# wangtong627/COR

Hardware: AMD Instinct MI355X
Metric: query triplets/sec (forward + similarity + top-k) (higher is better)
Workload: dtype bf16

## Files before the change

### cor_amd/csrc/flash_attn.hip

```cpp
#include <cstdlib>
#include <type_traits>

#include "common.h"

typedef short s16x4 __attribute__((ext_vector_type(4)));

namespace {

struct FlashArgs {
  const bf16_t* q; const bf16_t* k; const bf16_t* v; void* o;
  long q_sb, q_st, k_sb, k_st, v_sb, v_st, o_sb, o_st;
  int H, Tq, Tk;
  float scale_log2;
  float tbl_scale;
  const bf16_t* pad_row; const float* rel_h; const float* rel_w;
  int grid, S, nW, d3;
  int nqt;
  int rev;
};

constexpr int KT = 64;
constexpr int TILE_B = KT * 128;
constexpr int KV_BYTES = 4 * TILE_B;
constexpr int AUX_PER_WAVE = 8192;
// ... 717 lines not shown
  const int wi_ = a.rev ? (int)gridDim.x - 1 - wi0_ : wi0_;
  const int qt_ = wi_ % a.nqt, hb_ = wi_ / a.nqt;
  const int head = hb_ % a.H, b = hb_ / a.H;
  constexpr int S = 64;
  const int g2 = S * S;
  const bf16_t* kvbase = a.q + (long)b * g2 * a.d3 + head * 64;
  const int qh = qt_ * NW + wave;

  u32x4 qf[2][4];
#pragma unroll
  for (int qb = 0; qb < 2; ++qb) {
    const bf16_t* qp = a.q + ((long)b * g2 + qh * S + qb * 32 + r) * a.d3 + head * 64;
#pragma unroll
    for (int c = 0; c < 4; ++c) qf[qb][c] = *(const u32x4*)(qp + 16 * c + 8 * h);
  }

  float* aux = (float*)(smem + K_BYTES + V_BYTES + wave * AUXW);
  f32x16 wreg[2][2];
  {
    float* scr = (float*)(smem + wave * (3 * 4096));
    uint4 fh[2][4], fw[4][4];
#pragma unroll
    for (int kb = 0; kb < 2; ++kb)
#pragma unroll
      for (int c = 0; c < 4; ++c) fh[kb][c] = table_frag(a.rel_h, qh + (S - 1) - (kb * 32 + r), c, h);
#pragma unroll
    for (int jb = 0; jb < 4; ++jb)
#pragma unroll
      for (int c = 0; c < 4; ++c) fw[jb][c] = table_frag(a.rel_w, min(jb * 32 + r, 2 * S - 2), c, h);
#pragma unroll
    for (int qb = 0; qb < 2; ++qb) {
#pragma unroll
      for (int kb = 0; kb < 2; ++kb) {
        f32x16 acc;
#pragma unroll
        for (int e = 0; e < 16; ++e) acc[e] = 0.f;
#pragma unroll
        for (int c = 0; c < 4; ++c)
          acc = __builtin_amdgcn_mfma_f32_32x32x16_bf16(__builtin_bit_cast(bf16x8, fh[kb][c]), __builtin_bit_cast(bf16x8, qf[qb][c]), acc, 0, 0, 0);
#pragma unroll
        for (int e = 0; e < 16; ++e) aux[(kb * 32 + acc_row(e, h)) * 64 + qb * 32 + r] = acc[e] * a.tbl_scale;
      }
#pragma unroll
      for (int jb = 0; jb < 3; ++jb) {
        f32x16 acc;
#pragma unroll
        for (int e = 0; e < 16; ++e) acc[e] = 0.f;
#pragma unroll
        for (int c = 0; c < 4; ++c)
          acc = __builtin_amdgcn_mfma_f32_32x32x16_bf16(__builtin_bit_cast(bf16x8, fw[qb + jb][c]), __builtin_bit_cast(bf16x8, qf[qb][c]), acc, 0, 0, 0);
#pragma unroll
        for (int e = 0; e < 16; ++e) scr[(jb * 32 + acc_row(e, h)) * 32 + r] = acc[e] * a.tbl_scale;
      }
      __builtin_amdgcn_fence(__ATOMIC_ACQ_REL, "wavefront");
#pragma unroll
      for (int kb = 0; kb < 2; ++kb)
#pragma unroll
        for (int e = 0; e < 16; ++e) wreg[qb][kb][e] = scr[(r + (S - 1) - (kb * 32 + acc_row(e, h))) * 32 + r];
      __builtin_amdgcn_fence(__ATOMIC_ACQ_REL, "wavefront");
    }
  }
  __syncthreads();

  char* Kring = smem; char* Vring = smem + K_BYTES;
  const unsigned lds0 = __builtin_amdgcn_readfirstlane((unsigned)(size_t)((__attribute__((address_space(3))) char*)smem));
  const unsigned wofs = __builtin_amdgcn_readfirstlane(wave) * 1024u;
  const int nt = a.Tk / KT;
  const int srow = tid >> 3, sch = tid & 7;
  const int kswz = (sch ^ ((srow >> 1) & 7)) * 8;
  const int vswz = (sch ^ (((srow >> 1) & 1) << 2)) * 8;
  const unsigned vk0 = (unsigned)((srow * a.d3 + a.H * 64 + kswz) * 2), vk1 = vk0 + (unsigned)(32 * a.d3 * 2);
  const unsigned vv0 = (unsigned)((srow * a.d3 + 2 * a.H * 64 + vswz) * 2), vv1 = vv0 + (unsigned)(32 * a.d3 * 2);
  const long tile_bytes = (long)KT * a.d3 * 2;
  auto issue_k = [&](int t, int slot) {
    const char* base = (const char*)kvbase + (long)t * tile_bytes;
    const unsigned d = lds0 + slot * TILE_B + wofs;
    glds16_so(base, vk0, d);
    glds16_so(base, vk1, d + 4096);
  };
  auto issue_v = [&](int t, int slot) {
    const char* base = (const char*)kvbase + (long)t * tile_bytes;
    const unsigned d = lds0 + K_BYTES + slot * TILE_B + wofs;
    glds16_so(base, vv0, d);
    glds16_so(base, vv1, d + 4096);
  };
  issue_k(0, 0); issue_k(1, 1); issue_k(2, 2); issue_v(0, 0); issue_v(1, 1);
  *(uint4*)(Vring + 3 * TILE_B + tid * 16) = make_uint4(0, 0, 0, 0);
  *(uint4*)(Vring + 3 * TILE_B + 4096 + tid * 16) = make_uint4(0, 0, 0, 0);
  asm volatile("s_waitcnt vmcnt(0)" ::: "memory");
  __syncthreads();

  const int sw = (lane >> 1) & 7;
  int kch[4];
#pragma unroll
  for (int c = 0; c < 4; ++c) kch[c] = r * 128 + (((2 * c + h) ^ sw) << 4);
  const int v_tr = (4 * h + ((lane & 15) >> 2)) * 128 + (16 * ((lane >> 4) & 1) + 4 * (lane & 3)) * 2;
  const int v_trd[2] = {v_tr + ((lane >> 3) & 1) * 64, v_tr + (1 - ((lane >> 3) & 1)) * 64};

  f32x16 o[2][2], s[2][2];
  float lsum[2][2] = {{0.f, 0.f}, {0.f, 0.f}};
  float m[2] = {-INFINITY, -INFINITY};
  u32x4 pf[2][2][2];
#pragma unroll
  for (int qb = 0; qb < 2; ++qb)
#pragma unroll
    for (int x = 0; x < 2; ++x) {
#pragma unroll
      for (int e = 0; e < 16; ++e) o[qb][x][e] = 0.f;
      pf[qb][x][0] = u32x4{0, 0, 0, 0}; pf[qb][x][1] = u32x4{0, 0, 0, 0};
    }

  {
    uint4 kf[8];
#pragma unroll
    for (int i = 0; i < 8; ++i) kf[i] = *(const uint4*)(Kring + (i >> 2) * 32 * 128 + kch[i & 3]);
#pragma unroll
    for (int qb = 0; qb < 2; ++qb)
#pragma unroll
      for (int kb = 0; kb < 2; ++kb) {
        s[qb][kb] = wreg[qb][kb];
#pragma unroll
        for (int c = 0; c < 4; ++c)
          s[qb][kb] = __builtin_amdgcn_mfma_f32_32x32x16_bf16(__builtin_bit_cast(bf16x8, kf[kb * 4 + c]), __builtin_bit_cast(bf16x8, qf[qb][c]), s[qb][kb], 0, 0, 0);
      }
  }
  __syncthreads();

#pragma unroll
  for (int qb = 0; qb < 2; ++qb) {
#pragma unroll
    for (int c = 0; c < 4; ++c) asm volatile("" : "+a"(qf[qb][c]));
#pragma unroll
    for (int x = 0; x < 2; ++x) { asm volatile("" : "+v"(s[qb][x])); asm volatile("" : "+v"(wreg[qb][x])); asm volatile("" : "+a"(o[qb][x])); }
  }
  const char* ksrc = (const char*)kvbase + 3 * tile_bytes;
  const char* vsrc = (const char*)kvbase + 2 * tile_bytes;
  const unsigned vk0p = vk0 + 2048u, vk1p = vk1 - 2048u, vv0p = vv0 + 2048u, vv1p = vv1 - 2048u;

#pragma unroll 1
  for (int t = 0; t < nt; ++t) {
    auto dma_tile = [&](const unsigned dst, const unsigned v0, const unsigned v1, const char* src) __attribute__((always_inline)) {
      unsigned keep;
      asm volatile("s_mov_b32 %0, m0\n\ts_mov_b32 m0, %1\n\ts_nop 0\n\t"
                   "global_load_lds_dwordx4 %2, %4 offset:-2048\n\tglobal_load_lds_dwordx4 %3, %4 offset:2048\n\ts_mov_b32 m0, %0"
                   : "=&s"(keep) : "s"(dst), "v"(v0), "v"(v1), "s"(src) : "memory");
    };
    const unsigned kd = lds0 + (unsigned)((t + 3) & 3) * TILE_B + wofs + 2048u;
    const unsigned vd = lds0 + K_BYTES + (unsigned)((t + 2) & 3) * TILE_B + wofs + 2048u;
    const char *ksrc_t = ksrc, *vsrc_t = vsrc;
    if (t + 4 < nt) ksrc += tile_bytes;
    if (t + 3 < nt) vsrc += tile_bytes;
    if (!(DBG & 1) && (DBG & 512)) { dma_tile(kd, vk0p, vk1p, ksrc_t); dma_tile(vd, vv0p, vv1p, vsrc_t); }
    const char *Vs = Vring + ((t + 3) & 3) * TILE_B, *Ks = Kring + ((t + 1) & 3) * TILE_B;
    const float rh0 = aux[t * 64 + r], rh1 = aux[t * 64 + 32 + r];
    u32x4 vf[8], kf[8];
    if (DBG & 4) { Vs = Vring; Ks = Kring; }
#pragma unroll
    for (int i = 0; i < 8; ++i) {
      const int kb = i >> 2, ks = (i >> 1) & 1, db = i & 1;
      if ((DBG & 4) && t > 0) { vf[i] = u32x4{(unsigned)t, (unsigned)i, 3u, 4u}; continue; }
      const char* vb = Vs + (kb * 32 + ks * 16) * 128 + v_trd[db];
      const s16x4 v0 = __builtin_amdgcn_ds_read_tr16_b64_v4i16((__attribute__((address_space(3))) s16x4*)(vb));
      const s16x4 v1 = __builtin_amdgcn_ds_read_tr16_b64_v4i16((__attribute__((address_space(3))) s16x4*)(vb + 8 * 128));
      vf[i] = __builtin_bit_cast(u32x4, __builtin_shufflevector(v0, v1, 0, 1, 2, 3, 4, 5, 6, 7));
    }
#pragma unroll
    for (int i = 0; i < 8; ++i) {
      if ((DBG & 4) && t > 0) { kf[i] = u32x4{(unsigned)t, (unsigned)i, 1u, 2u}; continue; }
      kf[i] = *(const u32x4*)(Ks + (i >> 2) * 32 * 128 + kch[i & 3]);
    }
    __builtin_amdgcn_sched_barrier(0);

    auto pv = [&](int n) __attribute__((always_inline)) {
      const int qb = n >> 3, kb = (n >> 2) & 1, ks = (n >> 1) & 1, db = n & 1;
      if (DBG & 32) { asm volatile("" : "+a"(o[qb][db]) : "a"(vf[kb * 4 + ks * 2 + db]), "v"(pf[qb][kb][ks])); return; }
      asm volatile("v_mfma_f32_32x32x16_bf16 %0, %1, %2, %0" : "+a"(o[qb][db]) : "a"(vf[kb * 4 + ks * 2 + db]), "v"(pf[qb][kb][ks]));
    };
    auto qk = [&](int g, int c) __attribute__((always_inline)) {
      const int qb = g >> 1, kb = g & 1;
      if (DBG & 64) { asm volatile("" : "+v"(s[qb][kb]) : "a"(kf[kb * 4 + c]), "a"(qf[qb][c]), "v"(wreg[qb][kb])); return; }
      if (c == 0) asm volatile("v_mfma_f32_32x32x16_bf16 %0, %1, %2, %3" : "=&v"(s[qb][kb]) : "a"(kf[kb * 4 + c]), "a"(qf[qb][c]), "v"(wreg[qb][kb]));
      else asm volatile("v_mfma_f32_32x32x16_bf16 %0, %1, %2, %0" : "+v"(s[qb][kb]) : "a"(kf[kb * 4 + c]), "a"(qf[qb][c]));
    };
    float mloc[2];
#pragma unroll
    for (int qb = 0; qb < 2; ++qb) {
      float m4[4];
#pragma unroll
      for (int kb = 0; kb < 2; ++kb)
#pragma unroll
        for (int g = 0; g < 2; ++g) {
          const int e = 8 * g;
          const f32x16& x = s[qb][kb];
          if (DBG & 16) { m4[kb * 2 + g] = x[e]; continue; }
          const float t0 = max3f_(x[e], x[e + 1], x[e + 2]), t1 = max3f_(x[e + 3], x[e + 4], x[e + 5]);
          m4[kb * 2 + g] = max3f_(max3f_(t0, t1, x[e + 6]), x[e + 7], -INFINITY);
        }
      mloc[qb] = fmaxf(max3f_(m4[0], m4[1], m4[2]), m4[3]);
      __builtin_amdgcn_sched_barrier(0);
      pv(qb);
    }
    float msub[2], al0 = 1.f, al1 = 1.f;
    bool resc;
    {
      const float ml0 = fmaxf(mloc[0], other_half(mloc[0])) + rh0, ml1 = fmaxf(mloc[1], other_half(mloc[1])) + rh1;
      resc = __builtin_amdgcn_ballot_w64(ml0 > m[0] + 8.0f || ml1 > m[1] + 8.0f) != 0;
      if (resc) {
        const float mn0 = fmaxf(m[0], ml0), mn1 = fmaxf(m[1], ml1);
        al0 = __builtin_amdgcn_exp2f(m[0] - mn0); al1 = __builtin_amdgcn_exp2f(m[1] - mn1);
        m[0] = mn0; m[1] = mn1;
        lsum[0][0] *= al0; lsum[0][1] *= al0; lsum[1][0] *= al1; lsum[1][1] *= al1;
      }
      msub[0] = m[0] - rh0; msub[1] = m[1] - rh1;
    }
    __builtin_amdgcn_sched_barrier(0);
    float pe[4] = {0.f, 0.f, 0.f, 0.f};
#pragma unroll
    for (int c = 0; c <= 16; ++c) {
      float pn[4];
      uint32_t d0 = 0, d1 = 0;
      const int cp = c - 1, gp = cp >> 2, qbp = gp >> 1, kbp = gp & 1, k4 = cp & 3;
      if (c < 16) {
        const int g = c >> 2, qb = g >> 1, kb = g & 1, e0 = 4 * (c & 3);
#pragma unroll
        for (int i = 0; i < 2; ++i) pn[i] = (DBG & 8) ? s[qb][kb][e0 + i] - msub[qb] : (DBG & 256) ? __builtin_amdgcn_exp2f(s[qb][kb][e0 + i]) : __builtin_amdgcn_exp2f(s[qb][kb][e0 + i] - msub[qb]);
      }
      if (c > 0) { d0 = pk2(pe[0], pe[1]); if (!(DBG & 128)) lsum[qbp][k4 & 1] = sum2_bf16(d0, lsum[qbp][k4 & 1]); else if (c == 1) lsum[qbp][k4 & 1] += __uint_as_float(d0); }
      if (!(DBG & 1) && !(DBG & 512)) {
        if (c == 2) dma_tile(kd, vk0p, vk1p, ksrc_t);
        if (c == 10) dma_tile(vd, vv0p, vv1p, vsrc_t);
      }
      if (c < 4) pv(2 + 2 * c);
      else if (c < 8) pv(6 + c);
      else if (c < 10) pv(6 + c);
      else if (c < 12) qk(1, c - 8);
      else if (c < 16) qk(2, c - 12);
      __builtin_amdgcn_sched_barrier(0);
      if (c < 16) {
        const int g = c >> 2, qb = g >> 1, kb = g & 1, e0 = 4 * (c & 3);
#pragma unroll
        for (int i = 2; i < 4; ++i) pn[i] = (DBG & 8) ? s[qb][kb][e0 + i] - msub[qb] : (DBG & 256) ? __builtin_amdgcn_exp2f(s[qb][kb][e0 + i]) : __builtin_amdgcn_exp2f(s[qb][kb][e0 + i] - msub[qb]);
      }
      if (c > 0) {
        d1 = pk2(pe[2], pe[3]); if (!(DBG & 128)) lsum[qbp][k4 & 1] = sum2_bf16(d1, lsum[qbp][k4 & 1]);
        u32x4& dst = pf[qbp][kbp][k4 >> 1];
        if (k4 & 1) { dst[2] = d0; dst[3] = d1; } else { dst[0] = d0; dst[1] = d1; }
      }
      if (c < 4) pv(3 + 2 * c);
      else if (c < 8) qk(0, c - 4);
      else if (c < 10) qk(1, c - 8);
      else if (c == 16) { qk(3, 0); qk(3, 1); qk(3, 2); qk(3, 3); }
#pragma unroll
      for (int i = 0; i < 4; ++i) pe[i] = pn[i];
      __builtin_amdgcn_sched_barrier(0);
    }
    asm volatile("" :: "v"(lsum[0][0]), "v"(lsum[0][1]), "v"(lsum[1][0]), "v"(lsum[1][1]));
    if (resc) {
#pragma unroll
      for (int db = 0; db < 2; ++db)
#pragma unroll
        for (int e = 0; e < 16; ++e) {
          float x0 = o[0][db][e], x1 = o[1][db][e], t0, t1;
          asm volatile("v_accvgpr_read_b32 %2, %0\n\tv_accvgpr_read_b32 %3, %1\n\tv_mul_f32 %2, %2, %4\n\tv_mul_f32 %3, %3, %5\n\t"
                       "v_accvgpr_write_b32 %0, %2\n\tv_accvgpr_write_b32 %1, %3"
                       : "+a"(x0), "+a"(x1), "=&v"(t0), "=&v"(t1) : "v"(al0), "v"(al1));
          o[0][db][e] = x0; o[1][db][e] = x1;
        }
    }
    if (!(DBG & 2)) {
      asm volatile("s_waitcnt vmcnt(6)" ::: "memory");
      __syncthreads();
    }
  }
  {
    asm volatile("s_waitcnt vmcnt(0)" ::: "memory");
    const char* Vs = Vring + ((nt - 1) & 3) * TILE_B;
#pragma unroll
    for (int kb = 0; kb < 2; ++kb)
#pragma unroll
      for (int ks = 0; ks < 2; ++ks)
#pragma unroll
        for (int db = 0; db < 2; ++db) {
          const char* vb = Vs + (kb * 32 + ks * 16) * 128 + v_trd[db];
          const s16x4 v0 = __builtin_amdgcn_ds_read_tr16_b64_v4i16((__attribute__((address_space(3))) s16x4*)(vb));
          const s16x4 v1 = __builtin_amdgcn_ds_read_tr16_b64_v4i16((__attribute__((address_space(3))) s16x4*)(vb + 8 * 128));
          const u32x4 vfr = __builtin_bit_cast(u32x4, __builtin_shufflevector(v0, v1, 0, 1, 2, 3, 4, 5, 6, 7));
#pragma unroll
          for (int qb = 0; qb < 2; ++qb)
            asm volatile("v_mfma_f32_32x32x16_bf16 %0, %1, %2, %0" : "+a"(o[qb][db]) : "a"(vfr), "v"(pf[qb][kb][ks]));
        }
    asm volatile("s_nop 7\n\ts_nop 7\n\ts_nop 7\n\ts_nop 7" ::: "memory");
  }
#pragma unroll
  for (int qb = 0; qb < 2; ++qb) {
    const float l = lsum[qb][0] + lsum[qb][1];
    const float inv = 1.0f / (l + other_half(l));
    auto off = [&](int j) -> long { return ((long)b * g2 + qh * S + qb * 32 + j) * (long)(a.H * 64) + head * 64; };
    store_o_rows<TO, 64>(o[qb], inv, (char*)aux, (TO*)a.o, lane, off);
    __builtin_amdgcn_fence(__ATOMIC_ACQ_REL, "wavefront");
  }
}

constexpr int WIN_ROWS = 224, WIN_KV = WIN_ROWS * 128, WIN_T = 27 * 32 * 4, WIN_LDS = 2 * WIN_KV + 7 * WIN_T;

template <typename TO>
__global__ void __launch_bounds__(448, 4) win_attn(const FlashArgs a) {
  extern __shared__ __attribute__((aligned(16))) char smem[];
  const int tid = threadIdx.x, lane = tid & 63, wave = __builtin_amdgcn_readfirstlane(tid >> 6);
  const int r = lane & 31, h = lane >> 5;
  const int bid = a.rev ? (int)gridDim.x - 1 - (int)blockIdx.x : (int)blockIdx.x;
  const int head = bid % a.H, win = bid / a.H;
  const int nw2 = a.nW * a.nW, b = win / nw2, wi = win - b * nw2, wy = wi / a.nW, wx = wi - wy * a.nW;
  const int g2 = a.grid * a.grid;
  char* Kt = smem; char* Vt = smem + WIN_KV;
  float* T = (float*)(smem + 2 * WIN_KV + wave * WIN_T);

  {
    const unsigned lds0 = __builtin_amdgcn_readfirstlane((unsigned)(size_t)((__attribute__((address_space(3))) char*)smem));
    const int sl = lane & 7;
    long colp[2]; bool okx[2];
#pragma unroll
    for (int hf = 0; hf < 2; ++hf) {
      const int kw = min(8 * hf + (lane >> 3), 13), x = wx * 14 + kw;
      okx[hf] = x < a.grid;
      colp[hf] = ((long)b * g2 + x) * a.d3 + head * 64;
    }
#pragma unroll
    for (int i8 = 0; i8 < 8; ++i8) {
      const int i = wave * 8 + i8;
      const bool isv = i >= 28;
      const int ii = isv ? i - 28 : i, kh = ii >> 1, hf = ii & 1, y = wy * 14 + kh;
      const int chunk = isv ? (sl ^ (((lane >> 4) & 1) << 2)) : (sl ^ (4 * hf + (lane >> 4)));
      const long plane = (long)(isv ? 2 : 1) * a.H * 64 + chunk * 8;
      const bf16_t* src = (y < a.grid && okx[hf]) ? a.q + colp[hf] + (long)y * a.grid * a.d3 + plane : a.pad_row + head * 64 + plane;
      glds16(src, lds0 + (isv ? WIN_KV : 0) + ii * 1024);
    }
  }

  const int tq = min(wave * 32 + r, 195);
  const int qh = (tq * 4682) >> 16, qw = tq - 14 * qh;
  uint4 qf[4];
  {
    const int y = wy * 14 + qh, x = wx * 14 + qw;
    const bf16_t* qp = (y < a.grid && x < a.grid) ? a.q + ((long)b * g2 + (long)y * a.grid + x) * a.d3 + head * 64 : a.pad_row + head * 64;
#pragma unroll
    for (int c = 0; c < 4; ++c) qf[c] = *(const uint4*)(qp + 16 * c + 8 * h);
  }

  float colb[8];
  uint4 tf[2][4];
#pragma unroll
  for (int tbl = 0; tbl < 2; ++tbl)
#pragma unroll
    for (int c = 0; c < 4; ++c) tf[tbl][c] = table_frag(tbl == 0 ? a.rel_w : a.rel_h, min(r, 26), c, h);
#pragma unroll
  for (int tbl = 0; tbl < 2; ++tbl) {
    f32x16 acc;
#pragma unroll
    for (int e = 0; e < 16; ++e) acc[e] = 0.f;
#pragma unroll
    for (int c = 0; c < 4; ++c)
      acc = __builtin_amdgcn_mfma_f32_32x32x16_bf16(__builtin_bit_cast(bf16x8, tf[tbl][c]), __builtin_bit_cast(bf16x8, qf[c]), acc, 0, 0, 0);
#pragma unroll
    for (int e = 0; e < 16; ++e) {
      const int row = acc_row(e, h);
      if (row < 27) T[row * 32 + r] = acc[e] * a.tbl_scale;
    }
    __builtin_amdgcn_fence(__ATOMIC_ACQ_REL, "wavefront");
    if (tbl == 0) {
#pragma unroll
      for (int e8 = 0; e8 < 8; ++e8) {
        const int kw = (e8 & 3) + 8 * (e8 >> 2) + 4 * h;
        colb[e8] = kw < 14 ? T[(qw - min(kw, 13) + 13) * 32 + r] : -INFINITY;
      }
      __builtin_amdgcn_fence(__ATOMIC_ACQ_REL, "wavefront");
    }
  }

  if (a.scale_log2 != 1.0f) {
#pragma unroll
    for (int c = 0; c < 4; ++c) {
      uint32_t w[4] = {qf[c].x, qf[c].y, qf[c].z, qf[c].w};
#pragma unroll
      for (int i = 0; i < 4; ++i) w[i] = pk2(__uint_as_float(w[i] << 16) * a.scale_log2, __uint_as_float(w[i] & 0xffff0000u) * a.scale_log2);
      qf[c] = make_uint4(w[0], w[1], w[2], w[3]);
    }
  }

  asm volatile("s_waitcnt vmcnt(0)" ::: "memory");
  __syncthreads();

  const int sw = (r >> 1) & 7;
  const int k_rd = r * 128, v_tr = (4 * h + ((lane & 15) >> 2)) * 128 + (16 * ((lane >> 4) & 1) + 4 * (lane & 3)) * 2;
  const int v_trd[2] = {v_tr + ((lane >> 3) & 1) * 64, v_tr + (1 - ((lane >> 3) & 1)) * 64};
  const int t_rd = (qh + 13) * 32 + r;
  f32x16 o[2], lsum;
#pragma unroll
  for (int e = 0; e < 16; ++e) { o[0][e] = 0.f; o[1][e] = 0.f; lsum[e] = 0.f; }
  float m = 0.f;
  const uint4 ones = make_uint4(0x3F803F80u, 0x3F803F80u, 0x3F803F80u, 0x3F803F80u);
#pragma unroll
  for (int blk = 0; blk < 7; ++blk) {
    const char* Kb = Kt + blk * 32 * 128 + k_rd;
    uint4 kf[4];
#pragma unroll
    for (int c = 0; c < 4; ++c) kf[c] = *(const uint4*)(Kb + (((2 * c + h) ^ sw) << 4));
    const float rm0 = T[t_rd - 32 * (2 * blk)] - m, rm1 = T[t_rd - 32 * (2 * blk + 1)] - m;
    f32x16 s;
#pragma unroll
    for (int e = 0; e < 16; ++e) s[e] = colb[e & 7] + (e < 8 ? rm0 : rm1);
#pragma unroll
    for (int c = 0; c < 4; ++c)
      s = __builtin_amdgcn_mfma_f32_32x32x16_bf16(__builtin_bit_cast(bf16x8, kf[c]), __builtin_bit_cast(bf16x8, qf[c]), s, 0, 0, 0);
    float mloc = max3f_(max3f_(s[0], s[1], s[2]), max3f_(s[3], s[4], s[5]), max3f_(s[6], s[7], s[8]));
    mloc = fmaxf(max3f_(mloc, max3f_(s[9], s[10], s[11]), max3f_(s[12], s[13], s[14])), s[15]);
    mloc = fmaxf(mloc, other_half(mloc));
    if (blk == 0 || __builtin_amdgcn_ballot_w64(mloc > 8.0f) != 0) {
      const float d = blk == 0 ? mloc : fmaxf(mloc, 0.f);
      const float alpha = __builtin_amdgcn_exp2f(-d);
      m += d;
#pragma unroll
      for (int e = 0; e < 16; ++e) s[e] -= d;
      if (blk != 0) {
        lsum[1] *= alpha; lsum[2] *= alpha;
#pragma unroll
        for (int e = 0; e < 16; ++e) { o[0][e] *= alpha; o[1][e] *= alpha; }
      }
    }
    uint4 pf[2];
    {
      f32x16 p;
#pragma unroll
      for (int e = 0; e < 16; ++e) p[e] = __builtin_amdgcn_exp2f(s[e]);
      pf[0] = pack8(p[0], p[1], p[2], p[3], p[4], p[5], p[6], p[7]);
      pf[1] = pack8(p[8], p[9], p[10], p[11], p[12], p[13], p[14], p[15]);
      lsum[1] = sum2_bf16(pf[0].y, sum2_bf16(pf[0].x, lsum[1])); lsum[2] = sum2_bf16(pf[0].w, sum2_bf16(pf[0].z, lsum[2]));
      lsum[1] = sum2_bf16(pf[1].y, sum2_bf16(pf[1].x, lsum[1])); lsum[2] = sum2_bf16(pf[1].w, sum2_bf16(pf[1].z, lsum[2]));
    }
#pragma unroll
    for (int ks = 0; ks < 2; ++ks) {
#pragma unroll
      for (int db = 0; db < 2; ++db) {
        const char* vb = Vt + (blk * 32 + ks * 16) * 128 + v_trd[db];
        const s16x4 v0 = __builtin_amdgcn_ds_read_tr16_b64_v4i16((__attribute__((address_space(3))) s16x4*)(vb));
        const s16x4 v1 = __builtin_amdgcn_ds_read_tr16_b64_v4i16((__attribute__((address_space(3))) s16x4*)(vb + 8 * 128));
        const uint2 u0 = __builtin_bit_cast(uint2, v0), u1 = __builtin_bit_cast(uint2, v1);
        const uint4 vfr = make_uint4(u0.x, u0.y, u1.x, u1.y);
        o[db] = __builtin_amdgcn_mfma_f32_32x32x16_bf16(__builtin_bit_cast(bf16x8, vfr), __builtin_bit_cast(bf16x8, pf[ks]), o[db], 0, 0, 0);
      }
    }
  }

  const float lhalf = lsum[1] + lsum[2];
  const float inv = 1.0f / (lhalf + other_half(lhalf));
  char* stg = (char*)T;
  TO* out = (TO*)a.o;
  auto off = [&](int jq) -> long {
    const int tj = wave * 32 + jq;
    if (tj >= 196) return -1;
    const int jh = (tj * 4682) >> 16, y = wy * 14 + jh, x = wx * 14 + (tj - 14 * jh);
    if (y >= a.grid || x >= a.grid) return -1;
    return ((long)b * g2 + (long)y * a.grid + x) * (long)(a.H * 64) + head * 64;
  };
  const long e0 = off(lane >> 2), e1 = off((lane >> 2) + 16);
  const int rd0 = (lane >> 2) * 80 + (lane & 3) * 16;
  __builtin_amdgcn_fence(__ATOMIC_ACQ_REL, "wavefront");
  if constexpr (sizeof(TO) == 2) {
#pragma unroll
    for (int db = 0; db < 2; ++db) {
#pragma unroll
      for (int g = 0; g < 4; ++g) {
        uint2 u;
        u.x = pk2(o[db][4 * g] * inv, o[db][4 * g + 1] * inv); u.y = pk2(o[db][4 * g + 2] * inv, o[db][4 * g + 3] * inv);
        *(uint2*)(stg + r * 80 + (8 * g + 4 * h) * 2) = u;
      }
      __builtin_amdgcn_fence(__ATOMIC_ACQ_REL, "wavefront");
      const uint4 v0 = *(const uint4*)(stg + rd0), v1 = *(const uint4*)(stg + rd0 + 16 * 80);
      if (e0 >= 0) *(uint4*)(out + e0 + db * 32 + (lane & 3) * 8) = v0;
      if (e1 >= 0) *(uint4*)(out + e1 + db * 32 + (lane & 3) * 8) = v1;
      __builtin_amdgcn_fence(__ATOMIC_ACQ_REL, "wavefront");
    }
  } else {
#pragma unroll
    for (int qd = 0; qd < 4; ++qd) {
      const int db = qd >> 1, g0 = 2 * (qd & 1);
#pragma unroll
      for (int gg = 0; gg < 2; ++gg) {
        const int g = g0 + gg;
        const f32x4 v4 = {o[db][4 * g] * inv, o[db][4 * g + 1] * inv, o[db][4 * g + 2] * inv, o[db][4 * g + 3] * inv};
        *(f32x4*)(stg + r * 80 + (8 * gg + 4 * h) * 4) = v4;
      }
      __builtin_amdgcn_fence(__ATOMIC_ACQ_REL, "wavefront");
      const f32x4 v0 = *(const f32x4*)(stg + rd0), v1 = *(const f32x4*)(stg + rd0 + 16 * 80);
      if (e0 >= 0) *(f32x4*)(out + e0 + qd * 16 + (lane & 3) * 4) = v0;
      if (e1 >= 0) *(f32x4*)(out + e1 + qd * 16 + (lane & 3) * 4) = v1;
      __builtin_amdgcn_fence(__ATOMIC_ACQ_REL, "wavefront");
    }
  }
}

template <typename TO>
int launch_win(const FlashArgs& a, int nwin, hipStream_t s) {
  static DevOnce once;
  cor_max_dyn_lds((const void*)win_attn<TO>, WIN_LDS, once);
  hipLaunchKernelGGL((win_attn<TO>), dim3(nwin * a.H), dim3(448), WIN_LDS, s, a);
  COR_CHECK_LAUNCH();
  return 0;
}

template <typename TO, bool STAMP = false, bool CB = false>
int launch_global_pipe(const FlashArgs& a, int nb, hipStream_t s) {
  const size_t lds = 6 * TILE_B + 4 * AUX_PER_WAVE;
  static DevOnce once;
  cor_max_dyn_lds((const void*)flash_global_pipe<TO, STAMP, CB>, (int)lds, once);
  FlashArgs b = a;
  b.nqt = cdiv(a.Tq, 128);
  hipLaunchKernelGGL((flash_global_pipe<TO, STAMP, CB>), dim3(b.nqt * a.H * nb), dim3(256), lds, s, b);
  COR_CHECK_LAUNCH();
  return 0;
}

template <typename TO, int DBG = 0>
int launch_global_w64(const FlashArgs& a, int nb, hipStream_t s) {
  const size_t lds = 8 * TILE_B + 4 * 64 * 64 * 4;
  static DevOnce once;
  cor_max_dyn_lds((const void*)flash_global_w64<TO, DBG>, (int)lds, once);
  FlashArgs b = a;
  b.nqt = a.Tq / 256;
  hipLaunchKernelGGL((flash_global_w64<TO, DBG>), dim3(b.nqt * a.H * nb), dim3(256), lds, s, b);
  COR_CHECK_LAUNCH();
  return 0;
}

template <int MODE, typename TO, int HD = 64>
int launch(const FlashArgs& a, int nb, hipStream_t s) {
  constexpr int ROWB = HD == 64 ? 128 : 208;
  const size_t lds = 4 * KT * ROWB + (MODE == 0 ? 0 : 4 * AUX_PER_WAVE);
  static DevOnce once;
  cor_max_dyn_lds((const void*)flash_fwd<MODE, TO, HD>, (int)lds, once);
  FlashArgs b = a;
  b.nqt = cdiv(a.Tq, 128);
  hipLaunchKernelGGL((flash_fwd<MODE, TO, HD>), dim3(b.nqt * a.H * nb), dim3(256), lds, s, b);
  COR_CHECK_LAUNCH();
  return 0;
}
template <int MODE, int HD>
int launch_t(const FlashArgs& a, int nb, int out_dtype, hipStream_t s) {
  if (out_dtype == COR_BF16) return launch<MODE, bf16_t, HD>(a, nb, s);
  if (out_dtype == COR_F32) return launch<MODE, float, HD>(a, nb, s);
  return COR_ENOSUPPORT;
}

}

int cor_flash_plain_bf16(const void* q, long q_sb, long q_st, const void* k, long k_sb, long k_st, const void* v, long v_sb, long v_st,
                         void* out, long o_sb, long o_st, int out_dtype, int B, int H, int Tq, int Tk, int hd, float scale, hipStream_t s) {
  if ((q_st | k_st | v_st | q_sb | k_sb | v_sb) & 7) return COR_ENOSUPPORT;
  if (((uintptr_t)q | (uintptr_t)k | (uintptr_t)v | (uintptr_t)out) & 15) return COR_ENOSUPPORT;
  if ((o_st | o_sb) & 7) return COR_ENOSUPPORT;
  FlashArgs a{};
  a.q = (const bf16_t*)q; a.k = (const bf16_t*)k; a.v = (const bf16_t*)v; a.o = out;
  a.q_sb = q_sb; a.q_st = q_st; a.k_sb = k_sb; a.k_st = k_st; a.v_sb = v_sb; a.v_st = v_st; a.o_sb = o_sb; a.o_st = o_st;
  a.H = H; a.Tq = Tq; a.Tk = Tk; a.scale_log2 = scale * LOG2E; a.tbl_scale = LOG2E; a.S = 1; a.grid = 1; a.nW = 1;
  if (hd == 64) return launch_t<0, 64>(a, B, out_dtype, s);
  if (hd == 72) return launch_t<0, 72>(a, B, out_dtype, s);
  if (hd == 80) return launch_t<0, 80>(a, B, out_dtype, s);
  return COR_ENOSUPPORT;
}

int cor_flash_sam_bf16(const void* qkv, void* out, int out_dtype, const void* pad_row, const float* rel_h, const float* rel_w, int B,
                       int H, int hd, int grid, int window, float q_prescale, int variant, hipStream_t s) {
  if (hd != 64 && hd != 80) return COR_ENOSUPPORT;
  const int rev = (variant & COR_ORDER_REVERSE) ? 1 : 0;
  variant &= ~COR_ORDER_REVERSE;
#ifdef COR_PROBES
  if (variant != 0 && variant != 1 && variant != 2 && variant != 4 && variant != 9 && !(variant >= 16 && variant < 4096)) return COR_EINVAL;
#else
  if (variant != 0 && variant != 1 && variant != 2 && variant != 4) return COR_EINVAL;
#endif
  if (((uintptr_t)qkv & 15) || ((uintptr_t)out & 15) || ((uintptr_t)rel_h & 15) || ((uintptr_t)rel_w & 15)) return COR_ENOSUPPORT;
  FlashArgs a{};
  a.q = (const bf16_t*)qkv; a.o = out; a.H = H; a.rev = rev;
  a.scale_log2 = LOG2E / sqrtf((float)hd) / q_prescale; a.tbl_scale = LOG2E / q_prescale;
  if (hd == 64 && fabsf(a.scale_log2 - 1.0f) < 1e-6f) { a.scale_log2 = 1.0f; a.tbl_scale = 8.0f; }
  a.pad_row = (const bf16_t*)pad_row; a.rel_h = rel_h; a.rel_w = rel_w; a.grid = grid; a.d3 = 3 * H * hd;
  if (window == 0) {
    if (grid != 64) return COR_ENOSUPPORT;
    a.S = 64; a.Tq = a.Tk = grid * grid; a.nW = 1;
#ifdef COR_PROBES
    if (const char* e = getenv("COR_ATTN_TK")) a.Tk = atoi(e);
#endif
    if (hd == 80) return launch_t<1, 80>(a, B, out_dtype, s);
#ifdef COR_PROBES
    if (variant >= 16 && out_dtype == COR_BF16 && a.scale_log2 == 1.0f) {
      switch (variant - 16) {
        case 1: return launch_global_w64<bf16_t, 1>(a, B, s);
        case 2: return launch_global_w64<bf16_t, 2>(a, B, s);
        case 3: return launch_global_w64<bf16_t, 3>(a, B, s);
        case 4: return launch_global_w64<bf16_t, 4>(a, B, s);
        case 8: return launch_global_w64<bf16_t, 8>(a, B, s);
        case 16: return launch_global_w64<bf16_t, 16>(a, B, s);
        case 32: return launch_global_w64<bf16_t, 32>(a, B, s);
        case 64: return launch_global_w64<bf16_t, 64>(a, B, s);
        case 96: return launch_global_w64<bf16_t, 96>(a, B, s);
        case 7: return launch_global_w64<bf16_t, 7>(a, B, s);
        case 127: return launch_global_w64<bf16_t, 127>(a, B, s);
        case 128: return launch_global_w64<bf16_t, 128>(a, B, s);
        case 256: return launch_global_w64<bf16_t, 256>(a, B, s);
        case 384: return launch_global_w64<bf16_t, 384>(a, B, s);
        case 512: return launch_global_w64<bf16_t, 512>(a, B, s);
        default: return COR_EINVAL;
      }
    }
    if (variant == 9) {
      if (out_dtype == COR_BF16) return launch_global_pipe<bf16_t, true>(a, B, s);
      if (out_dtype == COR_F32) return launch_global_pipe<float, true>(a, B, s);
    }
#endif
    if (variant == 4 && a.scale_log2 == 1.0f) {
      if (out_dtype == COR_BF16) return launch_global_w64<bf16_t>(a, B, s);
      if (out_dtype == COR_F32) return launch_global_w64<float>(a, B, s);
    }
    if (variant == 0 && a.scale_log2 == 1.0f) {
      if (out_dtype == COR_BF16) return launch_global_pipe<bf16_t, false, true>(a, B, s);
      if (out_dtype == COR_F32) return launch_global_pipe<float, false, true>(a, B, s);
    }
    if (variant == 0 || variant == 2 || variant == 4) {
      if (out_dtype == COR_BF16) return launch_global_pipe<bf16_t>(a, B, s);
      if (out_dtype == COR_F32) return launch_global_pipe<float>(a, B, s);
    }
    if (out_dtype == COR_BF16) return launch<1, bf16_t>(a, B, s);
    if (out_dtype == COR_F32) return launch<1, float>(a, B, s);
    return COR_ENOSUPPORT;
  }
  if (window != 14 || ((uintptr_t)pad_row & 15)) return COR_ENOSUPPORT;
  a.S = 14; a.Tq = a.Tk = 196; a.nW = (grid + 13) / 14;
  if (hd == 80) return launch_t<2, 80>(a, B * a.nW * a.nW, out_dtype, s);
  if (variant != 1) {
    if (out_dtype == COR_BF16) return launch_win<bf16_t>(a, B * a.nW * a.nW, s);
    if (out_dtype == COR_F32) return launch_win<float>(a, B * a.nW * a.nW, s);
    return COR_ENOSUPPORT;
  }
  if (out_dtype == COR_BF16) return launch<2, bf16_t>(a, B * a.nW * a.nW, s);
  if (out_dtype == COR_F32) return launch<2, float>(a, B * a.nW * a.nW, s);
  return COR_ENOSUPPORT;
}
```

Baseline: 777.5.

## Add persistent double-buffered windowed attention kernel as default path

Splits the windowed SAM attention kernel into helpers and adds a persistent variant that launches one block per CU and loops over (window, head) items. While computing the current item, it prefetches the next item's K/V into a second LDS buffer and loads the next Q fragments into registers. Items that are fully padding skip the compute and store. This targets per-block launch overhead and exposed global-load latency, at the cost of doubled LDS, lower occupancy (2 blocks per CU) and a per-iteration barrier. The default window path (variants 0 and 4) now uses it; timing-stamp probe variants are also added.

After: 783.0 (median of 6 runs). Within noise of the previous version (+0.7%).

```diff
diff --git a/cor_amd/csrc/flash_attn.hip b/cor_amd/csrc/flash_attn.hip
--- a/cor_amd/csrc/flash_attn.hip
+++ b/cor_amd/csrc/flash_attn.hip
@@ -1043,57 +1043,47 @@
 }
 
 constexpr int WIN_ROWS = 224, WIN_KV = WIN_ROWS * 128, WIN_T = 27 * 32 * 4, WIN_LDS = 2 * WIN_KV + 7 * WIN_T;
-
-template <typename TO>
-__global__ void __launch_bounds__(448, 4) win_attn(const FlashArgs a) {
-  extern __shared__ __attribute__((aligned(16))) char smem[];
-  const int tid = threadIdx.x, lane = tid & 63, wave = __builtin_amdgcn_readfirstlane(tid >> 6);
-  const int r = lane & 31, h = lane >> 5;
-  const int bid = a.rev ? (int)gridDim.x - 1 - (int)blockIdx.x : (int)blockIdx.x;
-  const int head = bid % a.H, win = bid / a.H;
-  const int nw2 = a.nW * a.nW, b = win / nw2, wi = win - b * nw2, wy = wi / a.nW, wx = wi - wy * a.nW;
-  const int g2 = a.grid * a.grid;
-  char* Kt = smem; char* Vt = smem + WIN_KV;
-  float* T = (float*)(smem + 2 * WIN_KV + wave * WIN_T);
-
-  {
-    const unsigned lds0 = __builtin_amdgcn_readfirstlane((unsigned)(size_t)((__attribute__((address_space(3))) char*)smem));
-    const int sl = lane & 7;
-    long colp[2]; bool okx[2];
-#pragma unroll
-    for (int hf = 0; hf < 2; ++hf) {
-      const int kw = min(8 * hf + (lane >> 3), 13), x = wx * 14 + kw;
-      okx[hf] = x < a.grid;
-      colp[hf] = ((long)b * g2 + x) * a.d3 + head * 64;
-    }
-#pragma unroll
-    for (int i8 = 0; i8 < 8; ++i8) {
-      const int i = wave * 8 + i8;
-      const bool isv = i >= 28;
-      const int ii = isv ? i - 28 : i, kh = ii >> 1, hf = ii & 1, y = wy * 14 + kh;
-      const int chunk = isv ? (sl ^ (((lane >> 4) & 1) << 2)) : (sl ^ (4 * hf + (lane >> 4)));
-      const long plane = (long)(isv ? 2 : 1) * a.H * 64 + chunk * 8;
-      const bf16_t* src = (y < a.grid && okx[hf]) ? a.q + colp[hf] + (long)y * a.grid * a.d3 + plane : a.pad_row + head * 64 + plane;
-      glds16(src, lds0 + (isv ? WIN_KV : 0) + ii * 1024);
-    }
-  }
-
-  const int tq = min(wave * 32 + r, 195);
-  const int qh = (tq * 4682) >> 16, qw = tq - 14 * qh;
-  uint4 qf[4];
-  {
-    const int y = wy * 14 + qh, x = wx * 14 + qw;
-    const bf16_t* qp = (y < a.grid && x < a.grid) ? a.q + ((long)b * g2 + (long)y * a.grid + x) * a.d3 + head * 64 : a.pad_row + head * 64;
-#pragma unroll
-    for (int c = 0; c < 4; ++c) qf[c] = *(const uint4*)(qp + 16 * c + 8 * h);
-  }
-
-  float colb[8];
-  uint4 tf[2][4];
-#pragma unroll
-  for (int tbl = 0; tbl < 2; ++tbl)
-#pragma unroll
-    for (int c = 0; c < 4; ++c) tf[tbl][c] = table_frag(tbl == 0 ? a.rel_w : a.rel_h, min(r, 26), c, h);
+__device__ __forceinline__ long win_out_elems(const FlashArgs& a, int nitems) { return (long)(nitems / (a.H * a.nW * a.nW)) * a.grid * a.grid * a.H * 64; }
+
+struct WinItem { int b, wy, wx, head; };
+__device__ __forceinline__ WinItem win_item(const FlashArgs& a, int bid) {
+  WinItem it;
+  it.head = bid % a.H;
+  const int win = bid / a.H, nw2 = a.nW * a.nW;
+  it.b = win / nw2;
+  const int wi = win - it.b * nw2;
+  it.wy = wi / a.nW; it.wx = wi - it.wy * a.nW;
+  return it;
+}
+
+__device__ __forceinline__ void win_issue_kv(const FlashArgs& a, const WinItem& it, unsigned lds_kv, int wave, int lane) {
+  const int g2 = a.grid * a.grid, sl = lane & 7;
+  long colp[2]; bool okx[2];
+#pragma unroll
+  for (int hf = 0; hf < 2; ++hf) {
+    const int kw = min(8 * hf + (lane >> 3), 13), x = it.wx * 14 + kw;
+    okx[hf] = x < a.grid;
+    colp[hf] = ((long)it.b * g2 + x) * a.d3 + it.head * 64;
+  }
+#pragma unroll
+  for (int i8 = 0; i8 < 8; ++i8) {
+    const int i = wave * 8 + i8;
+    const bool isv = i >= 28;
+    const int ii = isv ? i - 28 : i, kh = ii >> 1, hf = ii & 1, y = it.wy * 14 + kh;
+    const int chunk = isv ? (sl ^ (((lane >> 4) & 1) << 2)) : (sl ^ (4 * hf + (lane >> 4)));
+    const long plane = (long)(isv ? 2 : 1) * a.H * 64 + chunk * 8;
+    const bf16_t* src = (y < a.grid && okx[hf]) ? a.q + colp[hf] + (long)y * a.grid * a.d3 + plane : a.pad_row + it.head * 64 + plane;
+    glds16(src, lds_kv + (isv ? WIN_KV : 0) + ii * 1024);
+  }
+}
+
+__device__ __forceinline__ const bf16_t* win_q_src(const FlashArgs& a, const WinItem& it, int qh, int qw, int h) {
+  const int y = it.wy * 14 + qh, x = it.wx * 14 + qw;
+  const bf16_t* qp = (y < a.grid && x < a.grid) ? a.q + ((long)it.b * a.grid * a.grid + (long)y * a.grid + x) * a.d3 : a.pad_row;
+  return qp + it.head * 64 + 8 * h;
+}
+
+__device__ __forceinline__ void win_tables(const FlashArgs& a, const uint4 (&tf)[2][4], uint4 (&qf)[4], float* T, int r, int h, int qw, float (&colb)[8]) {
 #pragma unroll
   for (int tbl = 0; tbl < 2; ++tbl) {
     f32x16 acc;
@@ -1117,7 +1107,6 @@
       __builtin_amdgcn_fence(__ATOMIC_ACQ_REL, "wavefront");
     }
   }
-
   if (a.scale_log2 != 1.0f) {
 #pragma unroll
     for (int c = 0; c < 4; ++c) {
@@ -1127,19 +1116,19 @@
       qf[c] = make_uint4(w[0], w[1], w[2], w[3]);
     }
   }
-
-  asm volatile("s_waitcnt vmcnt(0)" ::: "memory");
-  __syncthreads();
-
+}
+
+__device__ __forceinline__ void win_keys(const uint4 (&qf)[4], const float (&colb)[8], const char* Kt, const char* Vt, const float* T, int lane, int qh,
+                                         f32x16 (&o)[2], float& inv) {
+  const int r = lane & 31, h = lane >> 5;
   const int sw = (r >> 1) & 7;
   const int k_rd = r * 128, v_tr = (4 * h + ((lane & 15) >> 2)) * 128 + (16 * ((lane >> 4) & 1) + 4 * (lane & 3)) * 2;
   const int v_trd[2] = {v_tr + ((lane >> 3) & 1) * 64, v_tr + (1 - ((lane >> 3) & 1)) * 64};
   const int t_rd = (qh + 13) * 32 + r;
-  f32x16 o[2], lsum;
+  f32x16 lsum;
 #pragma unroll
   for (int e = 0; e < 16; ++e) { o[0][e] = 0.f; o[1][e] = 0.f; lsum[e] = 0.f; }
   float m = 0.f;
-  const uint4 ones = make_uint4(0x3F803F80u, 0x3F803F80u, 0x3F803F80u, 0x3F803F80u);
 #pragma unroll
   for (int blk = 0; blk < 7; ++blk) {
     const char* Kb = Kt + blk * 32 * 128 + k_rd;
@@ -1191,17 +1180,20 @@
       }
     }
   }
-
   const float lhalf = lsum[1] + lsum[2];
-  const float inv = 1.0f / (lhalf + other_half(lhalf));
-  char* stg = (char*)T;
+  inv = 1.0f / (lhalf + other_half(lhalf));
+}
+
+template <typename TO>
+__device__ __forceinline__ void win_store(const FlashArgs& a, const WinItem& it, const f32x16 (&o)[2], float inv, char* stg, int wave, int lane) {
+  const int r = lane & 31, h = lane >> 5;
   TO* out = (TO*)a.o;
   auto off = [&](int jq) -> long {
     const int tj = wave * 32 + jq;
     if (tj >= 196) return -1;
-    const int jh = (tj * 4682) >> 16, y = wy * 14 + jh, x = wx * 14 + (tj - 14 * jh);
+    const int jh = (tj * 4682) >> 16, y = it.wy * 14 + jh, x = it.wx * 14 + (tj - 14 * jh);
     if (y >= a.grid || x >= a.grid) return -1;
-    return ((long)b * g2 + (long)y * a.grid + x) * (long)(a.H * 64) + head * 64;
+    return ((long)it.b * a.grid * a.grid + (long)y * a.grid + x) * (long)(a.H * 64) + it.head * 64;
   };
   const long e0 = off(lane >> 2), e1 = off((lane >> 2) + 16);
   const int rd0 = (lane >> 2) * 80 + (lane & 3) * 16;
@@ -1240,11 +1232,166 @@
   }
 }
 
-template <typename TO>
+template <typename TO, bool STAMP = false>
+__global__ void __launch_bounds__(448, 4) win_attn(const FlashArgs a) {
+  extern __shared__ __attribute__((aligned(16))) char smem[];
+  const int tid = threadIdx.x, lane = tid & 63, wave = __builtin_amdgcn_readfirstlane(tid >> 6);
+  const int r = lane & 31, h = lane >> 5;
+  const int bid = a.rev ? (int)gridDim.x - 1 - (int)blockIdx.x : (int)blockIdx.x;
+  const WinItem it = win_item(a, bid);
+  char* Kt = smem; char* Vt = smem + WIN_KV;
+  float* T = (float*)(smem + 2 * WIN_KV + wave * WIN_T);
+  unsigned long long ts[6];
+  auto stamp = [&](int i) { if (STAMP) { __builtin_amdgcn_sched_barrier(0); ts[i] = __builtin_readcyclecounter(); __builtin_amdgcn_sched_barrier(0); } };
+  stamp(0);
+
+  win_issue_kv(a, it, __builtin_amdgcn_readfirstlane((unsigned)(size_t)((__attribute__((address_space(3))) char*)smem)), wave, lane);
+
+  const int tq = min(wave * 32 + r, 195);
+  const int qh = (tq * 4682) >> 16, qw = tq - 14 * qh;
+  uint4 qf[4];
+  {
+    const bf16_t* qp = win_q_src(a, it, qh, qw, h);
+#pragma unroll
+    for (int c = 0; c < 4; ++c) qf[c] = *(const uint4*)(qp + 16 * c);
+  }
+
+  float colb[8];
+  uint4 tf[2][4];
+#pragma unroll
+  for (int tbl = 0; tbl < 2; ++tbl)
+#pragma unroll
+    for (int c = 0; c < 4; ++c) tf[tbl][c] = table_frag(tbl == 0 ? a.rel_w : a.rel_h, min(r, 26), c, h);
+  win_tables(a, tf, qf, T, r, h, qw, colb);
+  stamp(1);
+
+  asm volatile("s_waitcnt vmcnt(0)" ::: "memory");
+  __syncthreads();
+  stamp(2);
+
+  f32x16 o[2];
+  float inv;
+  win_keys(qf, colb, Kt, Vt, T, lane, qh, o, inv);
+  if (STAMP) asm volatile("" :: "v"(o[0]), "v"(o[1]), "v"(inv));
+  stamp(3);
+  win_store<TO>(a, it, o, inv, (char*)T, wave, lane);
+  if (STAMP) {
+    stamp(4);
+    asm volatile("s_waitcnt vmcnt(0)" ::: "memory");
+    stamp(5);
+    unsigned long long* st = (unsigned long long*)((TO*)a.o + win_out_elems(a, (int)gridDim.x)) + ((long)blockIdx.x * 7 + wave) * 8;
+    if (lane == 0) {
+#pragma unroll
+      for (int i = 0; i < 6; ++i) st[i] = ts[i];
+    }
+  }
+}
+
+constexpr int WINP_LDS = 4 * WIN_KV + 7 * WIN_T;
+
+template <typename TO, bool STAMP = false>
+__global__ void __launch_bounds__(448, 2) win_attn_persist(const FlashArgs a, const int nitems) {
+  extern __shared__ __attribute__((aligned(16))) char smem[];
+  const int tid = threadIdx.x, lane = tid & 63, wave = __builtin_amdgcn_readfirstlane(tid >> 6);
+  const int r = lane & 31, h = lane >> 5;
+  const int nb = (int)gridDim.x;
+  float* T = (float*)(smem + 4 * WIN_KV + wave * WIN_T);
+  const unsigned lds0 = __builtin_amdgcn_readfirstlane((unsigned)(size_t)((__attribute__((address_space(3))) char*)smem));
+  const int tq = min(wave * 32 + r, 195);
+  const int qh = (tq * 4682) >> 16, qw = tq - 14 * qh;
+  unsigned long long tsum[6] = {0, 0, 0, 0, 0, 0}, ts[7];
+  auto stamp = [&](int i) { if (STAMP) { __builtin_amdgcn_sched_barrier(0); ts[i] = __builtin_readcyclecounter(); __builtin_amdgcn_sched_barrier(0); } };
+
+  int i = (int)blockIdx.x;
+  WinItem nxt = win_item(a, a.rev ? nitems - 1 - i : i);
+  win_issue_kv(a, nxt, lds0, wave, lane);
+  uint4 qf[4], tf[2][4];
+  {
+    const bf16_t* qp = win_q_src(a, nxt, qh, qw, h);
+#pragma unroll
+    for (int c = 0; c < 4; ++c) qf[c] = *(const uint4*)(qp + 16 * c);
+  }
+#pragma unroll
+  for (int tbl = 0; tbl < 2; ++tbl)
+#pragma unroll
+    for (int c = 0; c < 4; ++c) tf[tbl][c] = table_frag(tbl == 0 ? a.rel_w : a.rel_h, min(r, 26), c, h);
+  asm volatile("s_waitcnt vmcnt(0)" ::: "memory");
+#pragma unroll
+  for (int c = 0; c < 4; ++c) {
+    asm volatile("" : "+v"(qf[c].x), "+v"(qf[c].y), "+v"(qf[c].z), "+v"(qf[c].w));
+    asm volatile("" : "+v"(tf[0][c].x), "+v"(tf[0][c].y), "+v"(tf[0][c].z), "+v"(tf[0][c].w));
+    asm volatile("" : "+v"(tf[1][c].x), "+v"(tf[1][c].y), "+v"(tf[1][c].z), "+v"(tf[1][c].w));
+  }
+
+  for (int cur = 0; i < nitems; i += nb, cur ^= 1) {
+    stamp(0);
+    asm volatile("s_waitcnt lgkmcnt(0)" ::: "memory");
+    __builtin_amdgcn_s_barrier();
+    asm volatile("" ::: "memory");
+    stamp(1);
+    const WinItem it = nxt;
+    const bool more = i + nb < nitems;
+    uint4 qn[4];
+    if (more) {
+      nxt = win_item(a, a.rev ? nitems - 1 - (i + nb) : i + nb);
+      win_issue_kv(a, nxt, lds0 + (cur ^ 1) * (2 * WIN_KV), wave, lane);
+      const bf16_t* qp = win_q_src(a, nxt, qh, qw, h);
+#pragma unroll
+      for (int c = 0; c < 4; ++c) qn[c] = *(const uint4*)(qp + 16 * c);
+    }
+    stamp(2);
+    const bool live = __builtin_amdgcn_ballot_w64(it.wy * 14 + qh < a.grid && it.wx * 14 + qw < a.grid) != 0;
+    f32x16 o[2];
+    float inv;
+    if (live) {
+      float colb[8];
+      win_tables(a, tf, qf, T, r, h, qw, colb);
+      stamp(3);
+      const char* Kt = smem + cur * (2 * WIN_KV);
+      win_keys(qf, colb, Kt, Kt + WIN_KV, T, lane, qh, o, inv);
+      if (STAMP) asm volatile("" :: "v"(o[0]), "v"(o[1]), "v"(inv));
+    }
+    stamp(4);
+    if (more) {
+      asm volatile("s_waitcnt vmcnt(0)" ::: "memory");
+#pragma unroll
+      for (int c = 0; c < 4; ++c) {
+        asm volatile("" : "+v"(qn[c].x), "+v"(qn[c].y), "+v"(qn[c].z), "+v"(qn[c].w));
+        qf[c] = qn[c];
+      }
+    }
+    stamp(5);
+    if (live) win_store<TO>(a, it, o, inv, (char*)T, wave, lane);
+    stamp(6);
+    if (STAMP) {
+      tsum[0] += ts[1] - ts[0]; tsum[1] += ts[2] - ts[1]; tsum[4] += ts[5] - ts[4]; tsum[5] += ts[6] - ts[5];
+      if (live) { tsum[2] += ts[3] - ts[2]; tsum[3] += ts[4] - ts[3]; }
+    }
+  }
+  if (STAMP) {
+    unsigned long long* st = (unsigned long long*)((TO*)a.o + win_out_elems(a, nitems)) + ((long)blockIdx.x * 7 + wave) * 8;
+    if (lane == 0) {
+#pragma unroll
+      for (int k = 0; k < 6; ++k) st[k] = tsum[k];
+    }
+  }
+}
+
+template <typename TO, bool STAMP = false>
 int launch_win(const FlashArgs& a, int nwin, hipStream_t s) {
   static DevOnce once;
-  cor_max_dyn_lds((const void*)win_attn<TO>, WIN_LDS, once);
-  hipLaunchKernelGGL((win_attn<TO>), dim3(nwin * a.H), dim3(448), WIN_LDS, s, a);
+  cor_max_dyn_lds((const void*)win_attn<TO, STAMP>, WIN_LDS, once);
+  hipLaunchKernelGGL((win_attn<TO, STAMP>), dim3(nwin * a.H), dim3(448), WIN_LDS, s, a);
+  COR_CHECK_LAUNCH();
+  return 0;
+}
+
+template <typename TO, bool STAMP = false>
+int launch_win_persist(const FlashArgs& a, int nwin, hipStream_t s) {
+  static DevOnce once;
+  cor_max_dyn_lds((const void*)win_attn_persist<TO, STAMP>, WINP_LDS, once);
+  const int nitems = nwin * a.H;
+  hipLaunchKernelGGL((win_attn_persist<TO, STAMP>), dim3(min(nitems, cor_device_cus())), dim3(448), WINP_LDS, s, a, nitems);
   COR_CHECK_LAUNCH();
   return 0;
 }
@@ -1315,7 +1462,7 @@
   const int rev = (variant & COR_ORDER_REVERSE) ? 1 : 0;
   variant &= ~COR_ORDER_REVERSE;
 #ifdef COR_PROBES
-  if (variant != 0 && variant != 1 && variant != 2 && variant != 4 && variant != 9 && !(variant >= 16 && variant < 4096)) return COR_EINVAL;
+  if (variant != 0 && variant != 1 && variant != 2 && variant != 4 && variant != 9 && variant != 10 && !(variant >= 16 && variant < 4096)) return COR_EINVAL;
 #else
   if (variant != 0 && variant != 1 && variant != 2 && variant != 4) return COR_EINVAL;
 #endif
@@ -1377,11 +1524,22 @@
   if (window != 14 || ((uintptr_t)pad_row & 15)) return COR_ENOSUPPORT;
   a.S = 14; a.Tq = a.Tk = 196; a.nW = (grid + 13) / 14;
   if (hd == 80) return launch_t<2, 80>(a, B * a.nW * a.nW, out_dtype, s);
-  if (variant != 1) {
+#ifdef COR_PROBES
+  if (variant == 9 || variant == 10) {
+    if (out_dtype != COR_BF16) return COR_ENOSUPPORT;
+    return variant == 9 ? launch_win<bf16_t, true>(a, B * a.nW * a.nW, s) : launch_win_persist<bf16_t, true>(a, B * a.nW * a.nW, s);
+  }
+#endif
+  if (variant == 2) {
     if (out_dtype == COR_BF16) return launch_win<bf16_t>(a, B * a.nW * a.nW, s);
     if (out_dtype == COR_F32) return launch_win<float>(a, B * a.nW * a.nW, s);
     return COR_ENOSUPPORT;
   }
+  if (variant != 1) {
+    if (out_dtype == COR_BF16) return launch_win_persist<bf16_t>(a, B * a.nW * a.nW, s);
+    if (out_dtype == COR_F32) return launch_win_persist<float>(a, B * a.nW * a.nW, s);
+    return COR_ENOSUPPORT;
+  }
   if (out_dtype == COR_BF16) return launch<2, bf16_t>(a, B * a.nW * a.nW, s);
   if (out_dtype == COR_F32) return launch<2, float>(a, B * a.nW * a.nW, s);
   return COR_ENOSUPPORT;
```
